# jojolebarjos/board-game-simulator-python

Measured on AMD Instinct MI355X. Metric: env-steps/sec, Connect4(6,7,4) random rollout, batch=2^20 per GPU, higher is better.
Workload: dtype u64

## Files before the change

### board-game-simulator-python_amd/csrc/connect_kernels.hip

```cpp
#include <type_traits>

#include "bgs_common.h"
#include "bgs_internal.h"
#include "connect_board.h"

#ifndef BGS_TU_ID
#define BGS_TU_ID "unknown"
#endif
extern "C" const char bgs_tu_id_connect[] = BGS_TU_ID;

namespace bgs {
namespace {

template <int NW_, int SH, int SW, int SK>
struct Geo {
    static constexpr int NW = NW_;
    static constexpr int STATIC_H = SH, STATIC_W = SW, STATIC_K = SK;
    static constexpr int MAXW = SW ? SW : BGS_CONNECT_MAX_W;
    int rh, rw, rk;
    __device__ __forceinline__ int h() const { return SH ? SH : rh; }
    __device__ __forceinline__ int w() const { return SW ? SW : rw; }
    __device__ __forceinline__ int k() const { return SK ? SK : rk; }
    __device__ __forceinline__ uint32_t all_columns() const { return (1u << w()) - 1u; }
};

template <class G>
__device__ __forceinline__ bool ply_run_of_four(const G& g, uint64_t mine, uint32_t pos) {
    if constexpr (G::STATIC_H > 0 && G::STATIC_W > 0) {
        if constexpr (runs_start_low(G::STATIC_H, G::STATIC_W)) return four_in_a_row_at_low(mine, g.h(), pos);
        else return four_in_a_row_at(mine, g.h(), pos);
    } else {
        if (runs_start_low(g.h(), g.w())) return four_in_a_row_at_low(mine, g.h(), pos);
        return four_in_a_row_at(mine, g.h(), pos);
    }
}

__device__ __forceinline__ uint32_t four_in_a_row_low_hits(uint64_t b, int h) {
    const int dirs[3] = {h + 1, h + 2, h};
    uint32_t acc = 0;
#pragma unroll
    for (int d = 0; d < 3; ++d) {
        const uint64_t s1 = b >> dirs[d];
        const uint32_t pl = (uint32_t)b & (uint32_t)s1, ph = (uint32_t)(b >> 32) & (uint32_t)(s1 >> 32);
        uint32_t s2;
        asm("v_alignbit_b32 %0, %1, %2, %3" : "=v"(s2) : "v"(ph), "v"(pl), "s"(2 * dirs[d]));
        acc = d == 0 ? (pl & s2) : and_or(pl, s2, acc);
    }
    const uint64_t s1 = b >> 1;
    const uint32_t pl = (uint32_t)b & (uint32_t)s1, ph = (uint32_t)(b >> 32) & (uint32_t)(s1 >> 32);
    const uint64_t pairs = ((uint64_t)ph << 32) | pl;
    uint64_t s2;
    asm("v_lshrrev_b64 %0, %1, %2" : "=v"(s2) : "s"(2), "v"(pairs));
    return and_or(pl, (uint32_t)s2, acc) | (ph & (uint32_t)(s2 >> 32));
}

__device__ __forceinline__ int select_bit(uint32_t m, uint32_t i, int max_bits) {
    for (int j = 0; j + 1 < max_bits; ++j) {
        const uint32_t t = m & (m - 1u);
        m = ((uint32_t)j < i) ? t : m;
    }
    return __ffs((int)m) - 1;
}

template <int NW>
struct Lane {
    Bits<NW> cur, opp;
    uint64_t hts;
    uint32_t full;
    uint32_t plies;
};

template <class G>
__device__ __forceinline__ Lane<G::NW> empty_lane() {
    Lane<G::NW> l;
    l.cur = zero_bits<G::NW>();
    l.opp = zero_bits<G::NW>();
    l.hts = 0;
    l.full = 0;
    l.plies = 0;
    return l;
}

template <class G>
__device__ __forceinline__ Lane<G::NW> make_lane(const G& g, const Bits<G::NW>& p0, const Bits<G::NW>& p1) {
    Lane<G::NW> l;
    l.plies = popcount(p0) + popcount(p1);
    const bool second = l.plies & 1u;
    l.cur = second ? p1 : p0;
    l.opp = second ? p0 : p1;
    const Bits<G::NW> occ = p0 | p1;
    const int h = g.h(), w = g.w();
    const uint64_t colmask = (1ull << (h + 1)) - 1ull;
    l.hts = 0;
    l.full = 0;
#pragma unroll
    for (int x = 0; x < G::MAXW; ++x) {
        if (x < w) {
            const uint32_t hx = (uint32_t)__popcll(shr(occ, x * (h + 1)).w[0] & colmask);
            l.hts |= (uint64_t)hx << (4 * x);
            l.full |= (hx == (uint32_t)h) ? (1u << x) : 0u;
        }
    }
    return l;
}

template <class G>
__device__ __forceinline__ uint32_t drop_stone(const G& g, Lane<G::NW>& l, int col) {
    const int h = g.h();
    const uint32_t hx = (uint32_t)(l.hts >> (4 * col)) & 15u;
    set_bit(l.cur, col * (h + 1) + (int)hx);
    l.hts += 1ull << (4 * col);
    l.full |= (hx + 1u == (uint32_t)h) ? (1u << col) : 0u;
    const uint32_t mover = l.plies & 1u;
    const bool won = has_run(g, l.cur);
    const uint32_t st = won ? mover + 1u : (l.full == g.all_columns() ? BGS_ST_DRAW : BGS_ST_RUNNING);
// ... 547 lines not shown

    uint64_t p[2] = {0, 0};
    uint32_t hts = 0;
    uint32_t blk = 0;
    uint32_t live = 0;
    uint32_t st = 0;
    uint32_t game = 0;
    uint32_t skip = 0;
    uint32_t stepped = 0;

    if (avail == 0u) return;
    WaveCodes codes;
    if (CODES) codes.init(code_lds, games_per_wave, avail);
    do {
        const uint64_t need = __builtin_amdgcn_ballot_w64(live == 0);
        if (need && taken < avail) {
            const uint32_t rank = __builtin_amdgcn_mbcnt_hi((uint32_t)(need >> 32), __builtin_amdgcn_mbcnt_lo((uint32_t)need, 0u));
            if (live == 0 && taken + rank < avail) {
                game = taken + rank;
                st = 0;
                if (FROM_INITIAL) {
                    p[0] = 0;
                    p[1] = 0;
                    hts = top * columns;
                    blk = 0;
                    live = (!CAPPED || max_plies > 0u) ? ~0u : 0u;
                    if (CAPPED && live == 0) {
                        plane0[game] = 0;
                        plane1[game] = 0;
                        status_out[game] = 0;
                        reward_out[game] = 0;
                    }
                } else {
                    p[0] = plane0[game];
                    p[1] = plane1[game];
                    const uint32_t ply0 = (uint32_t)__popcll(p[0]) + (uint32_t)__popcll(p[1]);
                    const uint64_t occ = p[0] | p[1];
                    hts = 0;
#pragma unroll
                    for (int x = 0; x < G::MAXW; ++x) {
                        if (x < g.w() && x < 8) {
                            const uint32_t hx = (uint32_t)__popcll((occ >> (x * (int)stride)) & ((1ull << stride) - 1ull));
                            hts |= (top - hx) << (4 * x);
                        }
                    }
                    blk = ply0 >> 2;
                    skip = ply0 & 3u;
                    const uint32_t st0 = status_out[game];
                    live = (st0 == BGS_ST_RUNNING && (!CAPPED || ply0 < max_plies)) ? ~0u : 0u;
                    if (CODES && live == 0) codes.add(game, st0);
                }
            }
            const uint32_t wanted = (uint32_t)__popcll(need);
            taken = avail - taken < wanted ? avail : taken + wanted;
        }

        const uint32_t was_live = live;
        const BlockDraws<PER_PLY> draws(seed, first_game + (uint64_t)(begin + game), blk);
        uint32_t open = (hts >> 3) & ONES;
#pragma unroll
        for (uint32_t j = 0; j < 4; ++j) {
            const uint32_t cnt = (uint32_t)__popc(open);
            const uint32_t idx = sample_index(draws.draw(j), cnt);
            uint64_t cmp64, carry;
            asm("v_mad_u64_u32 %0, %1, %2, %3, %4" : "=v"(cmp64), "=s"(carry) : "v"(idx - open), "s"(ONES), "v"(eights));
            const uint32_t cmp = (uint32_t)cmp64;
            uint32_t col = (uint32_t)__popc(cmp & column_top);
            if (g.w() >= 8) col &= 7u;
            const uint32_t sh = col * 4u;
            const uint32_t v = (hts >> sh) & 15u;
            uint32_t base = col * stride + top;
            asm("" : "+v"(base));
            uint32_t pos = base - v;
            if ((uint32_t)g.w() * stride + top > 63u) pos &= 63u;
            const uint32_t act = (FROM_INITIAL || j >= skip) ? live : 0u;
            uint64_t& mine = p[j & 1u];
            const uint64_t bit = 1ull << pos;
            mine = ((uint64_t)and_or((uint32_t)(bit >> 32), act, (uint32_t)(mine >> 32)) << 32) |
                   and_or((uint32_t)bit, act, (uint32_t)mine);
            hts += act << sh;
            open = (hts >> 3) & ONES;
            bool won;
            if (g.k() == 4) {
                won = ply_run_of_four(g, mine, pos);
            } else {
                Bits<1> b;
                b.w[0] = mine;
                won = has_run(g, b);
            }
            stepped -= act;
            st = won ? (j & 1u) + 1u : st;
            live = (won || open == 0u) ? 0u : live;
            if (CAPPED) live = (4u * blk + j + 1u < max_plies) ? live : 0u;
        }
        blk += 1u;
        skip = 0;

        if (was_live != 0 && live == 0) {
            const uint32_t code = st ? st : (open == 0u ? BGS_ST_DRAW : BGS_ST_RUNNING);
            *reinterpret_cast<uint64_t*>(reinterpret_cast<char*>(plane0) + (game * 8u)) = p[0];
            *reinterpret_cast<uint64_t*>(reinterpret_cast<char*>(plane1) + (game * 8u)) = p[1];
            *(reinterpret_cast<uint8_t*>(status_out) + game) = (uint8_t)code;
            *reinterpret_cast<uint16_t*>(reinterpret_cast<char*>(reward_out) + (game * 2u)) = reward_pair(code);
            if (CODES) codes.add(game, code);
        }
    } while (__builtin_amdgcn_ballot_w64(live != 0) || taken < avail);
    if (CODES) codes.flush(codes_out, begin);
    add_steps(steps, stepped);
}

template <class G, int OPEN_BLOCKS, bool PER_PLY = false>
struct OpenedWords {
    static constexpr int LAST = G::STATIC_H > 0 ? (G::STATIC_H * G::STATIC_W + 3) / 4 - 1 : 11;
    static constexpr int COUNT = PER_PLY ? 1 : (LAST - OPEN_BLOCKS + 1 > 1 ? LAST - OPEN_BLOCKS + 1 : 1);
    static constexpr int QUADS = (COUNT + 3) / 4;
    static_assert(LAST <= 11 && OPEN_BLOCKS >= 1 && OPEN_BLOCKS <= 4, "three philox calls cover blocks 0 .. 11");
};

template <int QUADS>
struct OpenedPool {
    static constexpr uint32_t SLOTS = 64;
    uint64_t plane[2][SLOTS];
    uint32_t cols[SLOTS];
    uint4 words[QUADS][SLOTS];
};

constexpr uint32_t kReplayMark = 1u << 28;
constexpr uint32_t kReplayRow = 0x80000000u;

template <class G, int OPEN_BLOCKS, bool PER_PLY>
constexpr bool deferred_opening() {
    if constexpr (G::STATIC_H > 0 && G::STATIC_W > 0 && G::STATIC_K > 0)
        return !PER_PLY && kDeferredOpeningStages > 0 && OPEN_BLOCKS == kRolloutOpeningBlocks && kRolloutOpeningBlocks == 3 &&
               deferred_opening_ok(G::STATIC_H, G::STATIC_W, G::STATIC_K);
    else
        return false;
}

template <class G, class Pool>
__device__ __forceinline__ void open_games_deferred(const G& g, Pool& pool, uint32_t slot, uint64_t seed, uint64_t id, bool mine) {
    constexpr uint32_t ONES = 0x11111111u;
    const uint32_t top = (uint32_t)g.h() + 7u;
    const uint32_t columns = ONES & ((1u << (4 * g.w())) - 1u);
    const uint32_t stride = (uint32_t)g.h() + 1u;
    uint64_t q[2] = {0, 0};
    uint32_t h4 = top * columns;
    auto cheap_ply = [&](uint32_t j, uint32_t draw, bool wrap) {
        const uint32_t col = sample_index(draw, (uint32_t)g.w());
        const uint32_t sh = col * 4u;
        const uint32_t v = (h4 >> sh) & 15u;
        uint32_t pos = col * stride + top - v;
        if (wrap) pos &= 63u;
        q[j & 1u] |= 1ull << pos;
        h4 -= 1u << sh;
    };
    auto blind_block = [&](uint32_t word, bool wrap) -> bool {
        cheap_ply(0u, sub_draw<0>(word), wrap);
        cheap_ply(1u, sub_draw<1>(word), wrap);
        cheap_ply(2u, sub_draw<2>(word), wrap);
        const bool closed = ((h4 >> 3) & ONES) != columns;
        cheap_ply(3u, sub_draw<3>(word), wrap);
        return closed;
    };
    auto park = [&](uint32_t cols, const uint4& lo, const uint4& hi) {
        pool.plane[0][slot] = q[0];
        pool.plane[1][slot] = q[1];
        pool.cols[slot] = cols;
        pool.words[0][slot] = lo;
        pool.words[1][slot] = hi;
    };
    const Philox4 a = philox4x32_10(seed, id, 0u);
    cheap_ply(0u, sub_draw<0>(a.v[0]), false);
    cheap_ply(1u, sub_draw<1>(a.v[0]), false);
    cheap_ply(2u, sub_draw<2>(a.v[0]), false);
    cheap_ply(3u, sub_draw<3>(a.v[0]), false);
    uint32_t* const slot_words0 = reinterpret_cast<uint32_t*>(&pool.words[0][slot]);
    uint32_t* const slot_words1 = reinterpret_cast<uint32_t*>(&pool.words[1][slot]);
    slot_words0[0] = a.v[1]; slot_words0[1] = a.v[2]; slot_words0[2] = a.v[3];
    uint64_t id_after = id;
    asm volatile("" : "+v"(id_after) : : "memory");
    uint32_t word9, word10;
    {
        Philox4 c = philox4x32_10(seed, id_after, 2u);
        slot_words1[3] = c.v[0];
        word9 = c.v[1];
        word10 = c.v[2];
        asm volatile("" : "+v"(id_after), "+v"(word9), "+v"(word10) : : "memory");
    }
    {
        const Philox4 b = philox4x32_10(seed, id_after, 1u);
        slot_words0[3] = b.v[0];
        slot_words1[0] = b.v[1]; slot_words1[1] = b.v[2]; slot_words1[2] = b.v[3];
    }
    pool.plane[0][slot] = q[0];
    pool.plane[1][slot] = q[1];
    pool.cols[slot] = mine ? (h4 | kReplayMark) : 0u;
    asm volatile("" ::: "memory");
    blind_block(slot_words0[0], false);
    const bool closed = blind_block(slot_words0[1], false);
    const uint32_t hits = four_in_a_row_low_hits(q[0], g.h()) | four_in_a_row_low_hits(q[1], g.h());
    const bool clean = mine && !closed && hits == 0u;
    if (clean) {
        const uint4 lo = pool.words[0][slot], hi = pool.words[1][slot];
        park(h4, make_uint4(lo.z, lo.w, hi.x, hi.y), make_uint4(hi.z, hi.w, word9, word10));
    }
    if constexpr (kDeferredOpeningStages >= 2) {
        asm volatile("" ::: "memory");
        const bool closed2 = blind_block(slot_words0[0], true);
        const uint32_t hits2 = four_in_a_row_low_hits(q[0], g.h()) | four_in_a_row_low_hits(q[1], g.h());
        if (clean && !closed2 && hits2 == 0u) {
            const uint4 lo = pool.words[0][slot], hi = pool.words[1][slot];
            park(h4, make_uint4(lo.y, lo.z, lo.w, hi.x), make_uint4(hi.y, hi.z, hi.w, 0u));
        }
    }
}

template <class G, int OPEN_BLOCKS, bool CODES, bool PER_PLY>
__global__ void __launch_bounds__(BGS_BLOCK)
k_connect_rollout_opened(G g, uint64_t* __restrict__ planes, uint8_t* __restrict__ status, uint16_t* __restrict__ reward,
                         int64_t n, uint64_t seed, uint64_t first_game, unsigned long long* __restrict__ steps,
                         uint32_t games_per_wave, uint32_t* __restrict__ codes_out) {
    using OW = OpenedWords<G, OPEN_BLOCKS, PER_PLY>;
    constexpr int NWORDS = OW::QUADS * 4;
    using Pool = OpenedPool<OW::QUADS>;
    constexpr bool DEFER = deferred_opening<G, OPEN_BLOCKS, PER_PLY>();
    static_assert(!DEFER || NWORDS == 8, "a replayed game refills rows 5 .. 7 with the words of blocks 8 .. 10");
    extern __shared__ uint32_t code_lds[];
    __shared__ Pool pools[BGS_BLOCK / BGS_WAVE];
    __shared__ uint32_t lane_words[BGS_BLOCK / BGS_WAVE][NWORDS][BGS_WAVE];
    constexpr uint32_t ONES = 0x11111111u;
    const uint32_t top = (uint32_t)g.h() + 7u;
    const uint32_t columns = g.w() >= 8 ? ONES : (ONES & ((1u << (4 * g.w())) - 1u));
    const uint32_t stride = (uint32_t)g.h() + 1u;
    const uint32_t column_top = 8u * columns;
    const uint64_t eights = 0x88888888ull;

    const uint32_t wave = __builtin_amdgcn_readfirstlane(blockIdx.x * (BGS_BLOCK / BGS_WAVE) + (threadIdx.x >> 6));
    const uint32_t lane = threadIdx.x & 63u;
    const int64_t begin = (int64_t)wave * games_per_wave;
    const int64_t end = begin + games_per_wave < n ? begin + games_per_wave : n;
    const uint32_t avail = begin < end ? (uint32_t)(end - begin) : 0u;
    uint32_t taken = 0;
    uint32_t opened = 0;
    uint64_t* __restrict__ const plane0 = planes + begin;
    uint64_t* __restrict__ const plane1 = planes + n + begin;
    Pool& pool = pools[threadIdx.x >> 6];

    uint64_t p[2] = {0, 0};
    uint32_t hts = 0, live = 0, game = 0;
    bool anywon = false;
    uint32_t wnext = 0;
    uint32_t* const my_words = &lane_words[threadIdx.x >> 6][0][lane];
    uint32_t wrow = 0;
    uint32_t myblk = 0;

    if (avail == 0u) return;
    uint8_t* const outcome = reinterpret_cast<uint8_t*>(code_lds + (threadIdx.x >> 6) * (games_per_wave >> 2));
    for (uint32_t i = lane; i < ((avail + 3u) >> 2); i += BGS_WAVE) reinterpret_cast<uint32_t*>(outcome)[i] = 0u;
    __builtin_amdgcn_wave_barrier();

    auto full_ply = [&](auto j_tag, uint32_t draw, uint64_t (&q)[2], uint32_t& h4, uint32_t& op, uint32_t& alive,
                        bool& won_any) {
        constexpr uint32_t J = decltype(j_tag)::value;
        const uint32_t cnt = (uint32_t)__popc(op);
        const uint32_t idx = sample_index(draw, cnt);
        uint64_t cmp64;
        {
            uint64_t carry;
            asm("v_mad_u64_u32 %0, %1, %2, %3, %4" : "=v"(cmp64), "=s"(carry) : "v"(idx - op), "s"(ONES), "v"(eights));
        }
        const uint32_t cmp = (uint32_t)cmp64;
        uint32_t col = (uint32_t)__popc(cmp & column_top);
        if (g.w() >= 8) col &= 7u;
        const uint32_t sh = col * 4u;
        const uint32_t v = (h4 >> sh) & 15u;
        uint32_t base = col * stride + top;
        asm("" : "+v"(base));
        uint32_t pos = base - v;
        if ((uint32_t)g.w() * stride + top > 63u) pos &= 63u;
        const uint32_t act = alive;
        uint64_t& mine = q[J & 1u];
        const uint64_t bit = 1ull << pos;
        mine = ((uint64_t)and_or((uint32_t)(bit >> 32), act, (uint32_t)(mine >> 32)) << 32) |
               and_or((uint32_t)bit, act, (uint32_t)mine);
        h4 += act << sh;
        op = (h4 >> 3) & ONES;
        bool won;
        if (g.k() == 4) {
            won = ply_run_of_four(g, mine, pos);
        } else {
            Bits<1> b;
            b.w[0] = mine;
            won = has_run(g, b);
        }
        won_any = won_any || won;
        alive = (won || op == 0u) ? 0u : alive;
    };
    auto outcome_of = [&](const uint64_t (&q)[2], bool won_any) -> uint32_t {
        const uint32_t stones = (uint32_t)__popcll(q[0]) + (uint32_t)__popcll(q[1]);
        return connect_outcome_byte(stones, won_any);
    };
    auto cheap_ply = [&](uint32_t j, uint32_t draw, uint64_t (&q)[2], uint32_t& h4) {
        const uint32_t col = sample_index(draw, (uint32_t)g.w());
        const uint32_t sh = col * 4u;
        const uint32_t v = (h4 >> sh) & 15u;
        const uint32_t pos = col * stride + top - v;
        q[j & 1u] |= 1ull << pos;
        h4 -= 1u << sh;
    };
    auto refetch = [&](uint64_t lane_seed, uint64_t id) {
        if (wrow == (kReplayRow | 7u)) {
            if (live != 0u) {
                const Philox4 d = philox4x32_10(lane_seed, id, 2u);
                my_words[5 * BGS_WAVE] = d.v[0];
                my_words[6 * BGS_WAVE] = d.v[1];
                my_words[7 * BGS_WAVE] = d.v[2];
            }
            wrow = 5u;
        }
    };
    auto play_block = [&]() {
        const uint32_t was_live = live;
        Philox4 four = {{0u, 0u, 0u, 0u}};
        uint32_t word = 0u;
        if constexpr (PER_PLY) {
            four = philox4x32_10(seed, first_game + (uint64_t)(begin + game), myblk);
            myblk += 1u;
        } else if constexpr (DEFER) {
            word = wnext;
            if (__builtin_amdgcn_ballot_w64(wrow == (kReplayRow | 7u))) refetch(seed, first_game + (uint64_t)(begin + game));
            wnext = my_words[wrow * BGS_WAVE];
            const int32_t up = (int32_t)(wrow + 1u);
            wrow = (uint32_t)(up < NWORDS - 1 ? up : NWORDS - 1);
        } else {
            word = wnext;
            wnext = my_words[wrow * BGS_WAVE];
            wrow = wrow + 1u < (uint32_t)NWORDS - 1u ? wrow + 1u : (uint32_t)NWORDS - 1u;
        }
        uint32_t open = (hts >> 3) & ONES;
        full_ply(std::integral_constant<uint32_t, 0>{}, PER_PLY ? four.v[0] : sub_draw<0>(word), p, hts, open, live, anywon);
        full_ply(std::integral_constant<uint32_t, 1>{}, PER_PLY ? four.v[1] : sub_draw<1>(word), p, hts, open, live, anywon);
        full_ply(std::integral_constant<uint32_t, 2>{}, PER_PLY ? four.v[2] : sub_draw<2>(word), p, hts, open, live, anywon);
        full_ply(std::integral_constant<uint32_t, 3>{}, PER_PLY ? four.v[3] : sub_draw<3>(word), p, hts, open, live, anywon);
        if (was_live != 0 && live == 0) {
            *reinterpret_cast<uint64_t*>(reinterpret_cast<char*>(plane0) + (game * 8u)) = p[0];
            *reinterpret_cast<uint64_t*>(reinterpret_cast<char*>(plane1) + (game * 8u)) = p[1];
            outcome[game] = (uint8_t)outcome_of(p, anywon);
        }
    };
    auto take = [&](uint32_t which) {
        game = which;
        const uint32_t slot = which & (Pool::SLOTS - 1u);
        p[0] = pool.plane[0][slot];
        p[1] = pool.plane[1][slot];
        hts = pool.cols[slot];
        if constexpr (PER_PLY) {
            myblk = (uint32_t)OPEN_BLOCKS;
        } else {
#pragma unroll
            for (int k = 0; k < OW::QUADS; ++k) {
                const uint4 v = pool.words[k][slot];
                if (k == 0) wnext = v.x; else my_words[(4 * k) * BGS_WAVE] = v.x;
                my_words[(4 * k + 1) * BGS_WAVE] = v.y;
                my_words[(4 * k + 2) * BGS_WAVE] = v.z;
                my_words[(4 * k + 3) * BGS_WAVE] = v.w;
            }
        }
        wrow = DEFER ? 1u | ((hts << 3) & kReplayRow) : 1u;
        anywon = false;
        live = hts != 0u ? ~0u : 0u;
    };
    auto open_games = [&]() {
        const uint32_t og = opened + lane;
        const uint64_t id = first_game + (uint64_t)(begin + og);
        if constexpr (DEFER) {
            open_games_deferred(g, pool, og & (Pool::SLOTS - 1u), seed, id, og < avail);
            opened += 64u;
            return;
        }
        uint64_t q[2] = {0, 0};
        uint32_t h4 = top * columns, alive = ~0u, op = columns;
        bool won_any = false;
        uint32_t words[12];
        Philox4 own = philox4x32_10(seed, id, 0u);
        using J0 = std::integral_constant<uint32_t, 0>; using J1 = std::integral_constant<uint32_t, 1>;
        using J2 = std::integral_constant<uint32_t, 2>; using J3 = std::integral_constant<uint32_t, 3>;
#define BGS_DRAW_OF(JT, b) (PER_PLY ? own.v[JT::value] : sub_draw<JT::value>(words[b]))
        if constexpr (!PER_PLY) {
            words[0] = own.v[0]; words[1] = own.v[1]; words[2] = own.v[2]; words[3] = own.v[3];
#pragma unroll
            for (int c = 1; c < 3; ++c) {
                if (4 * c <= OW::LAST) {
                    const Philox4 d = philox4x32_10(seed, id, (uint32_t)c);
                    words[4 * c] = d.v[0]; words[4 * c + 1] = d.v[1]; words[4 * c + 2] = d.v[2]; words[4 * c + 3] = d.v[3];
                } else {
                    words[4 * c] = words[4 * c + 1] = words[4 * c + 2] = words[4 * c + 3] = 0u;
                }
            }
        } else {
#pragma unroll
            for (int c = 0; c < 12; ++c) words[c] = 0u;
        }
        cheap_ply(0u, BGS_DRAW_OF(J0, 0), q, h4);
        cheap_ply(1u, BGS_DRAW_OF(J1, 0), q, h4);
        cheap_ply(2u, BGS_DRAW_OF(J2, 0), q, h4);
        cheap_ply(3u, BGS_DRAW_OF(J3, 0), q, h4);
        if (OPEN_BLOCKS >= 2) {
            if constexpr (PER_PLY) own = philox4x32_10(seed, id, 1u);
            cheap_ply(0u, BGS_DRAW_OF(J0, 1), q, h4);
            cheap_ply(1u, BGS_DRAW_OF(J1, 1), q, h4);
            op = (h4 >> 3) & ONES;
            full_ply(J2{}, BGS_DRAW_OF(J2, 1), q, h4, op, alive, won_any);
            full_ply(J3{}, BGS_DRAW_OF(J3, 1), q, h4, op, alive, won_any);
        }
#pragma unroll
        for (int ob = 2; ob < OPEN_BLOCKS; ++ob) {
            if constexpr (PER_PLY) own = philox4x32_10(seed, id, (uint32_t)ob);
            full_ply(J0{}, BGS_DRAW_OF(J0, ob), q, h4, op, alive, won_any);
            full_ply(J1{}, BGS_DRAW_OF(J1, ob), q, h4, op, alive, won_any);
            full_ply(J2{}, BGS_DRAW_OF(J2, ob), q, h4, op, alive, won_any);
            full_ply(J3{}, BGS_DRAW_OF(J3, ob), q, h4, op, alive, won_any);
        }
#undef BGS_DRAW_OF
        if (OPEN_BLOCKS >= 2 && og < avail && alive == 0) {
            plane0[og] = q[0];
            plane1[og] = q[1];
            outcome[og] = (uint8_t)outcome_of(q, won_any);
        }
        const uint32_t slot = og & (Pool::SLOTS - 1u);
        pool.plane[0][slot] = q[0];
        pool.plane[1][slot] = q[1];
        pool.cols[slot] = alive ? h4 : 0u;
#pragma unroll
        for (int k = 0; k < OW::QUADS; ++k) {
            auto at = [&](int i) { return OPEN_BLOCKS + i <= 11 ? words[OPEN_BLOCKS + i <= 11 ? OPEN_BLOCKS + i : 11] : 0u; };
            pool.words[k][slot] = make_uint4(at(4 * k), at(4 * k + 1), at(4 * k + 2), at(4 * k + 3));
        }
        opened += 64u;
    };

    while (taken < avail) {
        const uint64_t need = __builtin_amdgcn_ballot_w64(live == 0);
        if (need) {
            const uint32_t wanted = (uint32_t)__popcll(need);
            const uint32_t rank = __builtin_amdgcn_mbcnt_hi((uint32_t)(need >> 32), __builtin_amdgcn_mbcnt_lo((uint32_t)need, 0u));
            const uint32_t have = opened - taken;
            if (wanted > have && opened < avail) {
                const bool first = live == 0 && rank < have;
                const bool second = live == 0 && !first;
                if (first && taken + rank < avail) take(taken + rank);
                __builtin_amdgcn_fence(__ATOMIC_ACQ_REL, "wavefront");
                __builtin_amdgcn_wave_barrier();
                open_games();
                __builtin_amdgcn_fence(__ATOMIC_ACQ_REL, "wavefront");
                __builtin_amdgcn_wave_barrier();
                if (second && taken + rank < avail) take(taken + rank);
            } else if (live == 0 && taken + rank < avail) {
                take(taken + rank);
            }
            taken = avail - taken < wanted ? avail : taken + wanted;
        }
        play_block();
    }
    while (__builtin_amdgcn_ballot_w64(live != 0)) play_block();

    __builtin_amdgcn_fence(__ATOMIC_ACQ_REL, "wavefront");
    __builtin_amdgcn_wave_barrier();
    uint8_t* __restrict__ const status_out = status + begin;
    uint16_t* __restrict__ const reward_out = reward + begin;
    uint8_t* __restrict__ const packed_out = reinterpret_cast<uint8_t*>(codes_out) + (begin >> 2);
    uint32_t stepped = 0;
    for (uint32_t g4 = lane * 4u; g4 < avail; g4 += BGS_WAVE * 4u) {
        const ConnectOutcome4 o = connect_outcome4(reinterpret_cast<const uint32_t*>(outcome)[g4 >> 2]);
        stepped += o.plies;
        if (CODES) packed_out[g4 >> 2] = (uint8_t)o.codes;
        if (g4 + 4u <= avail) {
            *reinterpret_cast<uint32_t*>(status_out + g4) = o.status;
            *reinterpret_cast<uint2*>(reward_out + g4) = make_uint2(o.reward[0], o.reward[1]);
        } else {
            for (uint32_t k = 0; g4 + k < avail; ++k) {
                status_out[g4 + k] = (uint8_t)(o.status >> (8u * k));
                reward_out[g4 + k] = (uint16_t)((((uint64_t)o.reward[1] << 32) | o.reward[0]) >> (16u * k));
            }
        }
    }
    add_steps(steps, stepped);
}

template <class G, int OPEN_BLOCKS, bool CODES>
__global__ void __launch_bounds__(BGS_BLOCK)
k_connect_rollout_opened_steps(G g, const ConnectGroup tab, int64_t n, uint32_t games_per_wave) {
    using OW = OpenedWords<G, OPEN_BLOCKS, false>;
    constexpr int NWORDS = OW::QUADS * 4;
    using Pool = OpenedPool<OW::QUADS>;
    constexpr bool DEFER = deferred_opening<G, OPEN_BLOCKS, false>();
    static_assert(!DEFER || NWORDS == 8, "a replayed game refills rows 5 .. 7 with the words of blocks 8 .. 10");
    extern __shared__ uint32_t code_lds[];
    __shared__ Pool pools[BGS_BLOCK / BGS_WAVE];
    __shared__ uint32_t lane_words[BGS_BLOCK / BGS_WAVE][NWORDS][BGS_WAVE];
    constexpr uint32_t ONES = 0x11111111u;
    const uint32_t top = (uint32_t)g.h() + 7u;
    const uint32_t columns = g.w() >= 8 ? ONES : (ONES & ((1u << (4 * g.w())) - 1u));
    const uint32_t stride = (uint32_t)g.h() + 1u;
    const uint32_t column_top = 8u * columns;
    const uint64_t eights = 0x88888888ull;

    const uint32_t wave = __builtin_amdgcn_readfirstlane(blockIdx.x * (BGS_BLOCK / BGS_WAVE) + (threadIdx.x >> 6));
    const uint32_t lane = threadIdx.x & 63u;
    const int64_t begin = (int64_t)wave * games_per_wave;
    const int64_t end = begin + games_per_wave < n ? begin + games_per_wave : n;
    const uint32_t avail = begin < end ? (uint32_t)(end - begin) : 0u;
    const uint32_t nsteps = (uint32_t)tab.count;
    uint32_t taken = 0, opened = 0;
    Pool& pool = pools[threadIdx.x >> 6];

    uint32_t cur = 0;
    bool pending = false;
    uint64_t cur_seed = tab.step[0].seed, cur_first = tab.step[0].first_game;
    uint64_t* cur_planes = tab.step[0].planes ? tab.step[0].planes + begin : nullptr;
    uint64_t* prev_planes = nullptr;
    uint64_t prev_seed = 0, prev_first = 0;

    uint64_t p[2] = {0, 0};
    uint32_t hts = 0, live = 0;
    uint32_t game = 0;
    uint32_t old = 0;
    bool anywon = false;
    uint32_t wnext = 0;
    uint32_t* const my_words = &lane_words[threadIdx.x >> 6][0][lane];
    uint32_t wrow = 0;

    if (avail == 0u) return;
    uint8_t* const outcome_bytes = reinterpret_cast<uint8_t*>(code_lds);
    const uint32_t slices_at = __builtin_amdgcn_readfirstlane((threadIdx.x >> 6) * 2u * games_per_wave);
    auto slice_at = [&](uint32_t s) { return slices_at + (s & 1u) * games_per_wave; };
    auto slice_of = [&](uint32_t s) { return outcome_bytes + slice_at(s); };
    uint32_t cur_at = slice_at(0u), prev_at = 0;
    auto zero_slice = [&](uint32_t s) {
        uint32_t* const w = reinterpret_cast<uint32_t*>(slice_of(s));
        for (uint32_t i = lane; i < ((avail + 3u) >> 2); i += BGS_WAVE) w[i] = 0u;
        __builtin_amdgcn_fence(__ATOMIC_ACQ_REL, "wavefront");
        __builtin_amdgcn_wave_barrier();
    };
    zero_slice(0u);

    auto full_ply = [&](auto j_tag, uint32_t draw, uint64_t (&q)[2], uint32_t& h4, uint32_t& op, uint32_t& alive,
                        bool& won_any) {
        constexpr uint32_t J = decltype(j_tag)::value;
        const uint32_t cnt = (uint32_t)__popc(op);
        const uint32_t idx = sample_index(draw, cnt);
        uint64_t cmp64;
        {
            uint64_t carry;
            asm("v_mad_u64_u32 %0, %1, %2, %3, %4" : "=v"(cmp64), "=s"(carry) : "v"(idx - op), "s"(ONES), "v"(eights));
        }
        const uint32_t cmp = (uint32_t)cmp64;
        uint32_t col = (uint32_t)__popc(cmp & column_top);
        if (g.w() >= 8) col &= 7u;
        const uint32_t sh = col * 4u;
        const uint32_t v = (h4 >> sh) & 15u;
        uint32_t base = col * stride + top;
        asm("" : "+v"(base));
        uint32_t pos = base - v;
        if ((uint32_t)g.w() * stride + top > 63u) pos &= 63u;
        const uint32_t act = alive;
        uint64_t& mine = q[J & 1u];
        const uint64_t bit = 1ull << pos;
        mine = ((uint64_t)and_or((uint32_t)(bit >> 32), act, (uint32_t)(mine >> 32)) << 32) |
               and_or((uint32_t)bit, act, (uint32_t)mine);
        h4 += act << sh;
        op = (h4 >> 3) & ONES;
        bool won;
        if (g.k() == 4) {
            won = ply_run_of_four(g, mine, pos);
        } else {
            Bits<1> b;
            b.w[0] = mine;
            won = has_run(g, b);
        }
        won_any = won_any || won;
        alive = (won || op == 0u) ? 0u : alive;
    };
    auto outcome_of = [&](const uint64_t (&q)[2], bool won_any) -> uint32_t {
        const uint32_t stones = (uint32_t)__popcll(q[0]) + (uint32_t)__popcll(q[1]);
        return connect_outcome_byte(stones, won_any);
    };
    auto cheap_ply = [&](uint32_t j, uint32_t draw, uint64_t (&q)[2], uint32_t& h4) {
        const uint32_t col = sample_index(draw, (uint32_t)g.w());
        const uint32_t sh = col * 4u;
        const uint32_t v = (h4 >> sh) & 15u;
        const uint32_t pos = col * stride + top - v;
        q[j & 1u] |= 1ull << pos;
        h4 -= 1u << sh;
    };
    auto refetch = [&]() {
        const bool at = wrow == (kReplayRow | 7u);
#pragma unroll
        for (uint32_t o = 0; o < 2u; ++o) {
            const bool here = at && live != 0u && old == o;
            if (__builtin_amdgcn_ballot_w64(here) == 0) continue;
            if (here) {
                const Philox4 d = philox4x32_10(o ? prev_seed : cur_seed,
                                                (o ? prev_first : cur_first) + (uint64_t)(begin + (game - (o ? prev_at : cur_at))), 2u);
                my_words[5 * BGS_WAVE] = d.v[0];
                my_words[6 * BGS_WAVE] = d.v[1];
                my_words[7 * BGS_WAVE] = d.v[2];
            }
        }
        if (at) wrow = 5u;
    };
    auto play_block = [&]() {
        const uint32_t was_live = live;
        const uint32_t word = wnext;
        if constexpr (DEFER) {
            if (__builtin_amdgcn_ballot_w64(wrow == (kReplayRow | 7u))) refetch();
            wnext = my_words[wrow * BGS_WAVE];
            const int32_t up = (int32_t)(wrow + 1u);
            wrow = (uint32_t)(up < NWORDS - 1 ? up : NWORDS - 1);
        } else {
            wnext = my_words[wrow * BGS_WAVE];
            wrow = wrow + 1u < (uint32_t)NWORDS - 1u ? wrow + 1u : (uint32_t)NWORDS - 1u;
        }
        uint32_t open = (hts >> 3) & ONES;
        full_ply(std::integral_constant<uint32_t, 0>{}, sub_draw<0>(word), p, hts, open, live, anywon);
        full_ply(std::integral_constant<uint32_t, 1>{}, sub_draw<1>(word), p, hts, open, live, anywon);
        full_ply(std::integral_constant<uint32_t, 2>{}, sub_draw<2>(word), p, hts, open, live, anywon);
        full_ply(std::integral_constant<uint32_t, 3>{}, sub_draw<3>(word), p, hts, open, live, anywon);
        if (was_live != 0 && live == 0) {
            if (cur_planes != nullptr || prev_planes != nullptr) {
                uint64_t* const planes = old ? prev_planes : cur_planes;
                if (planes) {
                    const uint32_t at = (game - (old ? prev_at : cur_at)) * 8u;
                    *reinterpret_cast<uint64_t*>(reinterpret_cast<char*>(planes) + at) = p[0];
                    *reinterpret_cast<uint64_t*>(reinterpret_cast<char*>(planes + n) + at) = p[1];
                }
            }
            outcome_bytes[game] = (uint8_t)outcome_of(p, anywon);
        }
    };
    auto take = [&](uint32_t which) {
        game = cur_at + which;
        old = 0u;
        const uint32_t slot = which & (Pool::SLOTS - 1u);
        p[0] = pool.plane[0][slot];
        p[1] = pool.plane[1][slot];
        hts = pool.cols[slot];
#pragma unroll
        for (int k = 0; k < OW::QUADS; ++k) {
            const uint4 v = pool.words[k][slot];
            if (k == 0) wnext = v.x; else my_words[(4 * k) * BGS_WAVE] = v.x;
            my_words[(4 * k + 1) * BGS_WAVE] = v.y;
            my_words[(4 * k + 2) * BGS_WAVE] = v.z;
            my_words[(4 * k + 3) * BGS_WAVE] = v.w;
        }
        wrow = DEFER ? 1u | ((hts << 3) & kReplayRow) : 1u;
        anywon = false;
        live = hts != 0u ? ~0u : 0u;
    };
    auto open_games = [&]() {
        const uint32_t og = opened + lane;
        const uint64_t id = cur_first + (uint64_t)(begin + og);
        if constexpr (DEFER) {
            open_games_deferred(g, pool, og & (Pool::SLOTS - 1u), cur_seed, id, og < avail);
            opened += 64u;
            return;
        }
        uint64_t q[2] = {0, 0};
        uint32_t h4 = top * columns, alive = ~0u, op = columns;
        bool won_any = false;
        uint32_t words[12];
        const Philox4 own = philox4x32_10(cur_seed, id, 0u);
        using J2 = std::integral_constant<uint32_t, 2>; using J3 = std::integral_constant<uint32_t, 3>;
        using J0 = std::integral_constant<uint32_t, 0>; using J1 = std::integral_constant<uint32_t, 1>;
        words[0] = own.v[0]; words[1] = own.v[1]; words[2] = own.v[2]; words[3] = own.v[3];
#pragma unroll
        for (int c = 1; c < 3; ++c) {
            if (4 * c <= OW::LAST) {
                const Philox4 d = philox4x32_10(cur_seed, id, (uint32_t)c);
                words[4 * c] = d.v[0]; words[4 * c + 1] = d.v[1]; words[4 * c + 2] = d.v[2]; words[4 * c + 3] = d.v[3];
            } else {
                words[4 * c] = words[4 * c + 1] = words[4 * c + 2] = words[4 * c + 3] = 0u;
            }
        }
        cheap_ply(0u, sub_draw<0>(words[0]), q, h4);
        cheap_ply(1u, sub_draw<1>(words[0]), q, h4);
        cheap_ply(2u, sub_draw<2>(words[0]), q, h4);
        cheap_ply(3u, sub_draw<3>(words[0]), q, h4);
        if (OPEN_BLOCKS >= 2) {
            cheap_ply(0u, sub_draw<0>(words[1]), q, h4);
            cheap_ply(1u, sub_draw<1>(words[1]), q, h4);
            op = (h4 >> 3) & ONES;
            full_ply(J2{}, sub_draw<2>(words[1]), q, h4, op, alive, won_any);
            full_ply(J3{}, sub_draw<3>(words[1]), q, h4, op, alive, won_any);
        }
#pragma unroll
        for (int ob = 2; ob < OPEN_BLOCKS; ++ob) {
            full_ply(J0{}, sub_draw<0>(words[ob]), q, h4, op, alive, won_any);
            full_ply(J1{}, sub_draw<1>(words[ob]), q, h4, op, alive, won_any);
            full_ply(J2{}, sub_draw<2>(words[ob]), q, h4, op, alive, won_any);
            full_ply(J3{}, sub_draw<3>(words[ob]), q, h4, op, alive, won_any);
        }
        if (OPEN_BLOCKS >= 2 && og < avail && alive == 0) {
            if (cur_planes) {
                cur_planes[og] = q[0];
                cur_planes[n + og] = q[1];
            }
            slice_of(cur)[og] = (uint8_t)outcome_of(q, won_any);
        }
        const uint32_t slot = og & (Pool::SLOTS - 1u);
        pool.plane[0][slot] = q[0];
        pool.plane[1][slot] = q[1];
        pool.cols[slot] = alive ? h4 : 0u;
#pragma unroll
        for (int k = 0; k < OW::QUADS; ++k) {
            auto at = [&](int i) { return OPEN_BLOCKS + i <= 11 ? words[OPEN_BLOCKS + i <= 11 ? OPEN_BLOCKS + i : 11] : 0u; };
            pool.words[k][slot] = make_uint4(at(4 * k), at(4 * k + 1), at(4 * k + 2), at(4 * k + 3));
        }
        opened += 64u;
    };
    auto flush = [&](uint32_t s) {
        __builtin_amdgcn_fence(__ATOMIC_ACQ_REL, "wavefront");
        __builtin_amdgcn_wave_barrier();
        const ConnectGroupStep& e = tab.step[s];
        const uint32_t* const outcome = reinterpret_cast<const uint32_t*>(slice_of(s));
        uint8_t* __restrict__ const status_out = e.status + begin;
        uint16_t* __restrict__ const reward_out = e.reward + begin;
        uint8_t* __restrict__ const packed_out = reinterpret_cast<uint8_t*>(e.codes) + (begin >> 2);
        uint32_t stepped = 0;
#pragma unroll 1
        for (uint32_t g4 = lane * 4u; g4 < avail; g4 += BGS_WAVE * 4u) {
            const ConnectOutcome4 o = connect_outcome4(outcome[g4 >> 2]);
            stepped += o.plies;
            if (CODES) packed_out[g4 >> 2] = (uint8_t)o.codes;
            if (e.planes) {
                if (g4 + 4u <= avail) {
                    *reinterpret_cast<uint32_t*>(status_out + g4) = o.status;
                    *reinterpret_cast<uint2*>(reward_out + g4) = make_uint2(o.reward[0], o.reward[1]);
                } else {
                    for (uint32_t k = 0; g4 + k < avail; ++k) {
                        status_out[g4 + k] = (uint8_t)(o.status >> (8u * k));
                        reward_out[g4 + k] = (uint16_t)((((uint64_t)o.reward[1] << 32) | o.reward[0]) >> (16u * k));
                    }
                }
            }
        }
        add_steps(e.steps, stepped);
    };
    auto flush_done = [&]() {
        if (pending && __builtin_amdgcn_ballot_w64(live != 0 && old != 0) == 0) {
            flush(cur - 1u);
            pending = false;
            prev_planes = nullptr;
        }
    };

    while (taken < avail || cur + 1u < nsteps) {
        const uint64_t need = __builtin_amdgcn_ballot_w64(live == 0);
        if (need) {
            const bool needy = live == 0;
            const uint32_t wanted = (uint32_t)__popcll(need);
            const uint32_t rank = __builtin_amdgcn_mbcnt_hi((uint32_t)(need >> 32), __builtin_amdgcn_mbcnt_lo((uint32_t)need, 0u));
            const uint32_t have = opened - taken;
            if (wanted > have && opened < avail) {
                const bool first = needy && rank < have;
                const bool second = needy && !first;
                if (first && taken + rank < avail) take(taken + rank);
                __builtin_amdgcn_fence(__ATOMIC_ACQ_REL, "wavefront");
                __builtin_amdgcn_wave_barrier();
                open_games();
                __builtin_amdgcn_fence(__ATOMIC_ACQ_REL, "wavefront");
                __builtin_amdgcn_wave_barrier();
                if (second && taken + rank < avail) take(taken + rank);
            } else if (needy && taken + rank < avail) {
                take(taken + rank);
            }
            const uint32_t served = avail - taken < wanted ? avail - taken : wanted;
            taken += served;
            if (served < wanted && cur + 1u < nsteps && !pending) {
                old = 1u;
                prev_planes = cur_planes;
                prev_seed = cur_seed;
                prev_first = cur_first;
                prev_at = cur_at;
                cur = __builtin_amdgcn_readfirstlane(cur + 1u);
                cur_at = slice_at(cur);
                pending = true;
                cur_seed = tab.step[cur].seed;
                cur_first = tab.step[cur].first_game;
// ... 965 lines not shown
```

### board-game-simulator-python_amd/csrc/connect_unit.h

```cpp
#pragma once

#include <stdint.h>

struct ConnectGeom {
    int h, w, k, nw;
};

constexpr int kRolloutOpeningBlocks = 3;
constexpr int kGamesPerLaneOneWord = 8;
constexpr int kGamesPerLane = 4;

constexpr bool runs_start_low(int h, int w) { return (w - 4) * (h + 1) + h - 1 <= 31; }

constexpr bool deferred_opening_ok(int h, int w, int k) {
    return k == 4 && w >= 4 && w <= 7 && h <= 8 && w * (h + 1) <= 64 && runs_start_low(h, w) && 2 * k - 1 > 4 && h > 4 &&
           h + 7 >= 12 && h * w <= 44;
}
constexpr int kDeferredOpeningStages = 2;

constexpr uint32_t kOutcomeRun = 64u;
constexpr uint32_t connect_outcome_byte(uint32_t stones, bool run) { return stones | (run ? kOutcomeRun : 0u); }
struct ConnectOutcome4 {
    uint32_t status;
    uint32_t reward[2];
    uint32_t codes;
    uint32_t plies;
};
constexpr ConnectOutcome4 connect_outcome4(uint32_t four) {
    constexpr uint32_t L = 0x01010101u;
    const uint32_t run = (four >> 6) & L, odd = four & L;
    const uint32_t game = ((four + 0x7F7F7F7Fu) >> 7) & L;
    const uint32_t low = game & ~(run & ~odd);
    const uint32_t high = game & ~(run & odd);
    const uint32_t status = low | (high << 1);
    const uint32_t won1 = low & ~high, won2 = high & ~low;
    const uint32_t a = (won1 & 1u) | ((won1 & 0x100u) << 8), b = (won2 & 1u) | ((won2 & 0x100u) << 8);
    const uint32_t c = ((won1 >> 16) & 1u) | ((won1 >> 8) & 0x10000u), d = ((won2 >> 16) & 1u) | ((won2 >> 8) & 0x10000u);
    return ConnectOutcome4{status,
                           {a * 0xFF01u | b * 0x01FFu, c * 0xFF01u | d * 0x01FFu},
                           (status & 3u) | ((status >> 6) & 0xCu) | ((status >> 12) & 0x30u) | ((status >> 18) & 0xC0u),
                           ((four & 0x3F3F3F3Fu) * L) >> 24};
}
struct ConnectOutcome {
    uint32_t status, reward, code, plies;
};
constexpr ConnectOutcome connect_outcome(uint32_t byte) {
    const ConnectOutcome4 o = connect_outcome4(byte & 255u);
    return ConnectOutcome{o.status, o.reward[0], o.codes, o.plies};
}

constexpr int kConnectGroupSteps = 4;
constexpr int kConnectGroupMax = 8;
constexpr int kConnectGroupMinCall = 48;

struct ConnectGroupStep {
    uint64_t seed;
    uint64_t first_game;
    uint64_t* planes;
    uint8_t* status;
    uint16_t* reward;
    uint32_t* codes;
    unsigned long long* steps;
};
struct ConnectGroup {
    ConnectGroupStep step[kConnectGroupMax];
    int count;
};
```

Measured before the change: 1045 billion.

## Re-encode column heights as biased upward nibbles to shorten per-ply drop math

Column-height nibbles now start at a bias and count upward, so the drop position is simply column*stride plus the nibble. The board planes are stored shifted by an offset and shifted back only when written to global memory. Liveness becomes a 0/1 value, so a stone is placed with a single shift-or instead of masked and_or pairs, and open columns are computed with one bitop3. The goal is fewer ALU instructions per ply in the hot rollout loops, at the cost of an offset bit layout that must still fit the 64-bit word and keep the low-run check valid.

```diff
diff --git a/board-game-simulator-python_amd/csrc/connect_kernels.hip b/board-game-simulator-python_amd/csrc/connect_kernels.hip
--- a/board-game-simulator-python_amd/csrc/connect_kernels.hip
+++ b/board-game-simulator-python_amd/csrc/connect_kernels.hip
@@ -24,13 +24,14 @@
     __device__ __forceinline__ uint32_t all_columns() const { return (1u << w()) - 1u; }
 };
 
-template <class G>
+template <bool OFFSET, class G>
 __device__ __forceinline__ bool ply_run_of_four(const G& g, uint64_t mine, uint32_t pos) {
     if constexpr (G::STATIC_H > 0 && G::STATIC_W > 0) {
-        if constexpr (runs_start_low(G::STATIC_H, G::STATIC_W)) return four_in_a_row_at_low(mine, g.h(), pos);
+        constexpr bool LOW = OFFSET ? offset_runs_start_low(G::STATIC_H, G::STATIC_W) : runs_start_low(G::STATIC_H, G::STATIC_W);
+        if constexpr (LOW) return four_in_a_row_at_low(mine, g.h(), pos);
         else return four_in_a_row_at(mine, g.h(), pos);
     } else {
-        if (runs_start_low(g.h(), g.w())) return four_in_a_row_at_low(mine, g.h(), pos);
+        if (OFFSET ? offset_runs_start_low(g.h(), g.w()) : runs_start_low(g.h(), g.w())) return four_in_a_row_at_low(mine, g.h(), pos);
         return four_in_a_row_at(mine, g.h(), pos);
     }
 }
@@ -744,7 +745,7 @@
             open = (hts >> 3) & ONES;
             bool won;
             if (g.k() == 4) {
-                won = ply_run_of_four(g, mine, pos);
+                won = ply_run_of_four<false>(g, mine, pos);
             } else {
                 Bits<1> b;
                 b.w[0] = mine;
@@ -790,6 +791,15 @@
 constexpr uint32_t kReplayMark = 1u << 28;
 constexpr uint32_t kReplayRow = 0x80000000u;
 
+__device__ __forceinline__ uint64_t stone_at(uint32_t alive01, uint32_t pos) { return (uint64_t)alive01 << pos; }
+
+__device__ __forceinline__ uint32_t open_columns(uint32_t nibbles, uint32_t columns) {
+    const uint32_t full = nibbles >> 3;
+    uint32_t r;
+    asm("v_bitop3_b32 %0, %1, %2, %1 bitop3:0xc" : "=v"(r) : "v"(full), "s"(columns));
+    return r;
+}
+
 template <class G, int OPEN_BLOCKS, bool PER_PLY>
 constexpr bool deferred_opening() {
     if constexpr (G::STATIC_H > 0 && G::STATIC_W > 0 && G::STATIC_K > 0)
@@ -801,26 +811,22 @@
 
 template <class G, class Pool>
 __device__ __forceinline__ void open_games_deferred(const G& g, Pool& pool, uint32_t slot, uint64_t seed, uint64_t id, bool mine) {
-    constexpr uint32_t ONES = 0x11111111u;
-    const uint32_t top = (uint32_t)g.h() + 7u;
-    const uint32_t columns = ONES & ((1u << (4 * g.w())) - 1u);
+    const uint32_t columns = connect_nibble_columns(g.w());
     const uint32_t stride = (uint32_t)g.h() + 1u;
     uint64_t q[2] = {0, 0};
-    uint32_t h4 = top * columns;
+    uint32_t h4 = connect_nibbles_start(g.h(), g.w());
     auto cheap_ply = [&](uint32_t j, uint32_t draw, bool wrap) {
         const uint32_t col = sample_index(draw, (uint32_t)g.w());
-        const uint32_t sh = col * 4u;
-        const uint32_t v = (h4 >> sh) & 15u;
-        uint32_t pos = col * stride + top - v;
+        uint32_t pos = connect_drop_position(h4, col, stride);
         if (wrap) pos &= 63u;
         q[j & 1u] |= 1ull << pos;
-        h4 -= 1u << sh;
+        h4 = connect_nibbles_after(h4, col, 1u);
     };
     auto blind_block = [&](uint32_t word, bool wrap) -> bool {
         cheap_ply(0u, sub_draw<0>(word), wrap);
         cheap_ply(1u, sub_draw<1>(word), wrap);
         cheap_ply(2u, sub_draw<2>(word), wrap);
-        const bool closed = ((h4 >> 3) & ONES) != columns;
+        const bool closed = (h4 & (8u * columns)) != 0u;
         cheap_ply(3u, sub_draw<3>(word), wrap);
         return closed;
     };
@@ -890,11 +896,13 @@
     extern __shared__ uint32_t code_lds[];
     __shared__ Pool pools[BGS_BLOCK / BGS_WAVE];
     __shared__ uint32_t lane_words[BGS_BLOCK / BGS_WAVE][NWORDS][BGS_WAVE];
-    constexpr uint32_t ONES = 0x11111111u;
-    const uint32_t top = (uint32_t)g.h() + 7u;
-    const uint32_t columns = g.w() >= 8 ? ONES : (ONES & ((1u << (4 * g.w())) - 1u));
+    constexpr uint32_t ONES = kNibbleOnes;
+    const uint32_t columns = connect_nibble_columns(g.w());
     const uint32_t stride = (uint32_t)g.h() + 1u;
     const uint32_t column_top = 8u * columns;
+    const uint32_t unshift = (uint32_t)connect_plane_offset(g.h());
+    const uint32_t idle_pos_max = connect_idle_position_max(g.h(), g.w());
+    const uint32_t ones = ONES;
     const uint64_t eights = 0x88888888ull;
 
     const uint32_t wave = __builtin_amdgcn_readfirstlane(blockIdx.x * (BGS_BLOCK / BGS_WAVE) + (threadIdx.x >> 6));
@@ -929,27 +937,20 @@
         uint64_t cmp64;
         {
             uint64_t carry;
-            asm("v_mad_u64_u32 %0, %1, %2, %3, %4" : "=v"(cmp64), "=s"(carry) : "v"(idx - op), "s"(ONES), "v"(eights));
+            asm("v_mad_u64_u32 %0, %1, %2, %3, %4" : "=v"(cmp64), "=s"(carry) : "v"(idx - op), "v"(ones), "s"(eights));
         }
         const uint32_t cmp = (uint32_t)cmp64;
         uint32_t col = (uint32_t)__popc(cmp & column_top);
         if (g.w() >= 8) col &= 7u;
-        const uint32_t sh = col * 4u;
-        const uint32_t v = (h4 >> sh) & 15u;
-        uint32_t base = col * stride + top;
-        asm("" : "+v"(base));
-        uint32_t pos = base - v;
-        if ((uint32_t)g.w() * stride + top > 63u) pos &= 63u;
-        const uint32_t act = alive;
+        uint32_t pos = connect_drop_position(h4, col, stride);
+        if (idle_pos_max > 63u) pos &= 63u;
         uint64_t& mine = q[J & 1u];
-        const uint64_t bit = 1ull << pos;
-        mine = ((uint64_t)and_or((uint32_t)(bit >> 32), act, (uint32_t)(mine >> 32)) << 32) |
-               and_or((uint32_t)bit, act, (uint32_t)mine);
-        h4 += act << sh;
-        op = (h4 >> 3) & ONES;
+        mine |= stone_at(alive, pos);
+        h4 = connect_nibbles_after(h4, col, alive);
+        op = open_columns(h4, columns);
         bool won;
         if (g.k() == 4) {
-            won = ply_run_of_four(g, mine, pos);
+            won = ply_run_of_four<true>(g, mine, pos);
         } else {
             Bits<1> b;
             b.w[0] = mine;
@@ -964,11 +965,8 @@
     };
     auto cheap_ply = [&](uint32_t j, uint32_t draw, uint64_t (&q)[2], uint32_t& h4) {
         const uint32_t col = sample_index(draw, (uint32_t)g.w());
-        const uint32_t sh = col * 4u;
-        const uint32_t v = (h4 >> sh) & 15u;
-        const uint32_t pos = col * stride + top - v;
-        q[j & 1u] |= 1ull << pos;
-        h4 -= 1u << sh;
+        q[j & 1u] |= 1ull << connect_drop_position(h4, col, stride);
+        h4 = connect_nibbles_after(h4, col, 1u);
     };
     auto refetch = [&](uint64_t lane_seed, uint64_t id) {
         if (wrow == (kReplayRow | 7u)) {
@@ -982,7 +980,7 @@
         }
     };
     auto play_block = [&]() {
-        const uint32_t was_live = live;
+        const bool was_live = live != 0u;
         Philox4 four = {{0u, 0u, 0u, 0u}};
         uint32_t word = 0u;
         if constexpr (PER_PLY) {
@@ -999,14 +997,14 @@
             wnext = my_words[wrow * BGS_WAVE];
             wrow = wrow + 1u < (uint32_t)NWORDS - 1u ? wrow + 1u : (uint32_t)NWORDS - 1u;
         }
-        uint32_t open = (hts >> 3) & ONES;
+        uint32_t open = open_columns(hts, columns);
         full_ply(std::integral_constant<uint32_t, 0>{}, PER_PLY ? four.v[0] : sub_draw<0>(word), p, hts, open, live, anywon);
         full_ply(std::integral_constant<uint32_t, 1>{}, PER_PLY ? four.v[1] : sub_draw<1>(word), p, hts, open, live, anywon);
         full_ply(std::integral_constant<uint32_t, 2>{}, PER_PLY ? four.v[2] : sub_draw<2>(word), p, hts, open, live, anywon);
         full_ply(std::integral_constant<uint32_t, 3>{}, PER_PLY ? four.v[3] : sub_draw<3>(word), p, hts, open, live, anywon);
-        if (was_live != 0 && live == 0) {
-            *reinterpret_cast<uint64_t*>(reinterpret_cast<char*>(plane0) + (game * 8u)) = p[0];
-            *reinterpret_cast<uint64_t*>(reinterpret_cast<char*>(plane1) + (game * 8u)) = p[1];
+        if (was_live && live == 0) {
+            *reinterpret_cast<uint64_t*>(reinterpret_cast<char*>(plane0) + (game * 8u)) = p[0] >> unshift;
+            *reinterpret_cast<uint64_t*>(reinterpret_cast<char*>(plane1) + (game * 8u)) = p[1] >> unshift;
             outcome[game] = (uint8_t)outcome_of(p, anywon);
         }
     };
@@ -1030,7 +1028,7 @@
         }
         wrow = DEFER ? 1u | ((hts << 3) & kReplayRow) : 1u;
         anywon = false;
-        live = hts != 0u ? ~0u : 0u;
+        live = hts != 0u ? 1u : 0u;
     };
     auto open_games = [&]() {
         const uint32_t og = opened + lane;
@@ -1041,7 +1039,7 @@
             return;
         }
         uint64_t q[2] = {0, 0};
-        uint32_t h4 = top * columns, alive = ~0u, op = columns;
+        uint32_t h4 = connect_nibbles_start(g.h(), g.w()), alive = 1u, op = columns;
         bool won_any = false;
         uint32_t words[12];
         Philox4 own = philox4x32_10(seed, id, 0u);
@@ -1071,7 +1069,7 @@
             if constexpr (PER_PLY) own = philox4x32_10(seed, id, 1u);
             cheap_ply(0u, BGS_DRAW_OF(J0, 1), q, h4);
             cheap_ply(1u, BGS_DRAW_OF(J1, 1), q, h4);
-            op = (h4 >> 3) & ONES;
+            op = open_columns(h4, columns);
             full_ply(J2{}, BGS_DRAW_OF(J2, 1), q, h4, op, alive, won_any);
             full_ply(J3{}, BGS_DRAW_OF(J3, 1), q, h4, op, alive, won_any);
         }
@@ -1085,8 +1083,8 @@
         }
 #undef BGS_DRAW_OF
         if (OPEN_BLOCKS >= 2 && og < avail && alive == 0) {
-            plane0[og] = q[0];
-            plane1[og] = q[1];
+            plane0[og] = q[0] >> unshift;
+            plane1[og] = q[1] >> unshift;
             outcome[og] = (uint8_t)outcome_of(q, won_any);
         }
         const uint32_t slot = og & (Pool::SLOTS - 1u);
@@ -1160,11 +1158,13 @@
     extern __shared__ uint32_t code_lds[];
     __shared__ Pool pools[BGS_BLOCK / BGS_WAVE];
     __shared__ uint32_t lane_words[BGS_BLOCK / BGS_WAVE][NWORDS][BGS_WAVE];
-    constexpr uint32_t ONES = 0x11111111u;
-    const uint32_t top = (uint32_t)g.h() + 7u;
-    const uint32_t columns = g.w() >= 8 ? ONES : (ONES & ((1u << (4 * g.w())) - 1u));
+    constexpr uint32_t ONES = kNibbleOnes;
+    const uint32_t columns = connect_nibble_columns(g.w());
     const uint32_t stride = (uint32_t)g.h() + 1u;
     const uint32_t column_top = 8u * columns;
+    const uint32_t unshift = (uint32_t)connect_plane_offset(g.h());
+    const uint32_t idle_pos_max = connect_idle_position_max(g.h(), g.w());
+    const uint32_t ones = ONES;
     const uint64_t eights = 0x88888888ull;
 
     const uint32_t wave = __builtin_amdgcn_readfirstlane(blockIdx.x * (BGS_BLOCK / BGS_WAVE) + (threadIdx.x >> 6));
@@ -1214,27 +1214,20 @@
         uint64_t cmp64;
         {
             uint64_t carry;
-            asm("v_mad_u64_u32 %0, %1, %2, %3, %4" : "=v"(cmp64), "=s"(carry) : "v"(idx - op), "s"(ONES), "v"(eights));
+            asm("v_mad_u64_u32 %0, %1, %2, %3, %4" : "=v"(cmp64), "=s"(carry) : "v"(idx - op), "v"(ones), "s"(eights));
         }
         const uint32_t cmp = (uint32_t)cmp64;
         uint32_t col = (uint32_t)__popc(cmp & column_top);
         if (g.w() >= 8) col &= 7u;
-        const uint32_t sh = col * 4u;
-        const uint32_t v = (h4 >> sh) & 15u;
-        uint32_t base = col * stride + top;
-        asm("" : "+v"(base));
-        uint32_t pos = base - v;
-        if ((uint32_t)g.w() * stride + top > 63u) pos &= 63u;
-        const uint32_t act = alive;
+        uint32_t pos = connect_drop_position(h4, col, stride);
+        if (idle_pos_max > 63u) pos &= 63u;
         uint64_t& mine = q[J & 1u];
-        const uint64_t bit = 1ull << pos;
-        mine = ((uint64_t)and_or((uint32_t)(bit >> 32), act, (uint32_t)(mine >> 32)) << 32) |
-               and_or((uint32_t)bit, act, (uint32_t)mine);
-        h4 += act << sh;
-        op = (h4 >> 3) & ONES;
+        mine |= stone_at(alive, pos);
+        h4 = connect_nibbles_after(h4, col, alive);
+        op = open_columns(h4, columns);
         bool won;
         if (g.k() == 4) {
-            won = ply_run_of_four(g, mine, pos);
+            won = ply_run_of_four<true>(g, mine, pos);
         } else {
             Bits<1> b;
             b.w[0] = mine;
@@ -1249,11 +1242,8 @@
     };
     auto cheap_ply = [&](uint32_t j, uint32_t draw, uint64_t (&q)[2], uint32_t& h4) {
         const uint32_t col = sample_index(draw, (uint32_t)g.w());
-        const uint32_t sh = col * 4u;
-        const uint32_t v = (h4 >> sh) & 15u;
-        const uint32_t pos = col * stride + top - v;
-        q[j & 1u] |= 1ull << pos;
-        h4 -= 1u << sh;
+        q[j & 1u] |= 1ull << connect_drop_position(h4, col, stride);
+        h4 = connect_nibbles_after(h4, col, 1u);
     };
     auto refetch = [&]() {
         const bool at = wrow == (kReplayRow | 7u);
@@ -1272,7 +1262,7 @@
         if (at) wrow = 5u;
     };
     auto play_block = [&]() {
-        const uint32_t was_live = live;
+        const bool was_live = live != 0u;
         const uint32_t word = wnext;
         if constexpr (DEFER) {
             if (__builtin_amdgcn_ballot_w64(wrow == (kReplayRow | 7u))) refetch();
@@ -1283,18 +1273,18 @@
             wnext = my_words[wrow * BGS_WAVE];
             wrow = wrow + 1u < (uint32_t)NWORDS - 1u ? wrow + 1u : (uint32_t)NWORDS - 1u;
         }
-        uint32_t open = (hts >> 3) & ONES;
+        uint32_t open = open_columns(hts, columns);
         full_ply(std::integral_constant<uint32_t, 0>{}, sub_draw<0>(word), p, hts, open, live, anywon);
         full_ply(std::integral_constant<uint32_t, 1>{}, sub_draw<1>(word), p, hts, open, live, anywon);
         full_ply(std::integral_constant<uint32_t, 2>{}, sub_draw<2>(word), p, hts, open, live, anywon);
         full_ply(std::integral_constant<uint32_t, 3>{}, sub_draw<3>(word), p, hts, open, live, anywon);
-        if (was_live != 0 && live == 0) {
+        if (was_live && live == 0) {
             if (cur_planes != nullptr || prev_planes != nullptr) {
                 uint64_t* const planes = old ? prev_planes : cur_planes;
                 if (planes) {
                     const uint32_t at = (game - (old ? prev_at : cur_at)) * 8u;
-                    *reinterpret_cast<uint64_t*>(reinterpret_cast<char*>(planes) + at) = p[0];
-                    *reinterpret_cast<uint64_t*>(reinterpret_cast<char*>(planes + n) + at) = p[1];
+                    *reinterpret_cast<uint64_t*>(reinterpret_cast<char*>(planes) + at) = p[0] >> unshift;
+                    *reinterpret_cast<uint64_t*>(reinterpret_cast<char*>(planes + n) + at) = p[1] >> unshift;
                 }
             }
             outcome_bytes[game] = (uint8_t)outcome_of(p, anywon);
@@ -1317,7 +1307,7 @@
         }
         wrow = DEFER ? 1u | ((hts << 3) & kReplayRow) : 1u;
         anywon = false;
-        live = hts != 0u ? ~0u : 0u;
+        live = hts != 0u ? 1u : 0u;
     };
     auto open_games = [&]() {
         const uint32_t og = opened + lane;
@@ -1328,7 +1318,7 @@
             return;
         }
         uint64_t q[2] = {0, 0};
-        uint32_t h4 = top * columns, alive = ~0u, op = columns;
+        uint32_t h4 = connect_nibbles_start(g.h(), g.w()), alive = 1u, op = columns;
         bool won_any = false;
         uint32_t words[12];
         const Philox4 own = philox4x32_10(cur_seed, id, 0u);
@@ -1351,7 +1341,7 @@
         if (OPEN_BLOCKS >= 2) {
             cheap_ply(0u, sub_draw<0>(words[1]), q, h4);
             cheap_ply(1u, sub_draw<1>(words[1]), q, h4);
-            op = (h4 >> 3) & ONES;
+            op = open_columns(h4, columns);
             full_ply(J2{}, sub_draw<2>(words[1]), q, h4, op, alive, won_any);
             full_ply(J3{}, sub_draw<3>(words[1]), q, h4, op, alive, won_any);
         }
@@ -1364,8 +1354,8 @@
         }
         if (OPEN_BLOCKS >= 2 && og < avail && alive == 0) {
             if (cur_planes) {
-                cur_planes[og] = q[0];
-                cur_planes[n + og] = q[1];
+                cur_planes[og] = q[0] >> unshift;
+                cur_planes[n + og] = q[1] >> unshift;
             }
             slice_of(cur)[og] = (uint8_t)outcome_of(q, won_any);
         }
diff --git a/board-game-simulator-python_amd/csrc/connect_unit.h b/board-game-simulator-python_amd/csrc/connect_unit.h
--- a/board-game-simulator-python_amd/csrc/connect_unit.h
+++ b/board-game-simulator-python_amd/csrc/connect_unit.h
@@ -17,6 +17,30 @@
            h + 7 >= 12 && h * w <= 44;
 }
 constexpr int kDeferredOpeningStages = 2;
+
+constexpr uint32_t kNibbleOnes = 0x11111111u;
+constexpr int connect_nibble_bias(int h) { return 8 - h; }
+constexpr int connect_plane_offset(int h) { return 8 - h; }
+constexpr uint32_t connect_nibble_columns(int w) { return w >= 8 ? kNibbleOnes : (kNibbleOnes & ((1u << (4 * w)) - 1u)); }
+constexpr uint32_t connect_nibbles_start(int h, int w) { return (uint32_t)connect_nibble_bias(h) * connect_nibble_columns(w); }
+constexpr bool offset_runs_start_low(int h, int w) { return (w - 4) * (h + 1) + h - 1 + connect_plane_offset(h) <= 31; }
+constexpr bool offset_fits_word(int h, int w) { return w * (h + 1) + connect_plane_offset(h) <= 64; }
+constexpr uint32_t connect_open_columns(uint32_t nibbles, uint32_t columns) { return columns & ~(nibbles >> 3); }
+constexpr uint32_t connect_nth_open_column(uint32_t open, uint32_t columns, uint32_t idx, int w) {
+    const uint32_t cmp = (idx - open) * kNibbleOnes + 0x88888888u;
+    const uint32_t col = (uint32_t)__builtin_popcount(cmp & (8u * columns));
+    return w >= 8 ? (col & 7u) : col;
+}
+constexpr uint32_t connect_drop_position(uint32_t nibbles, uint32_t col, uint32_t stride) {
+    return col * stride + ((nibbles >> (4u * col)) & 15u);
+}
+constexpr uint32_t connect_nibbles_after(uint32_t nibbles, uint32_t col, uint32_t alive01) {
+    return nibbles + (alive01 << (4u * col));
+}
+constexpr uint32_t connect_idle_position_max(int h, int w) {
+    const uint32_t sentinel = (uint32_t)((w - 1) * (h + 1) + 8), beyond = w >= 8 ? 0u : (uint32_t)(w * (h + 1) + 1);
+    return sentinel > beyond ? sentinel : beyond;
+}
 
 constexpr uint32_t kOutcomeRun = 64u;
 constexpr uint32_t connect_outcome_byte(uint32_t stones, bool run) { return stones | (run ? kOutcomeRun : 0u); }
```

Result: faster. 1079 billion (median of 5 runs) (+3.2%).
